# SuneelFreimuth/raytracer-server

Measured on NVIDIA B200. Metric: samples/sec (Mrays/sec alongside) on flying_unicorn, higher is better.
Workload: dtype f32

## Files before the change

### raytracer-server_b200/csrc/wavefront.cuh

```cuda
#pragma once

#include "adaptive_rule.cuh"
#include "intersect.cuh"
#include "octree.cuh"
#include "shade.cuh"

namespace rtb {

constexpr int WF_THREADS = 256;
constexpr int TILE = 32;
constexpr uint32_t SHADOW_PROBE = 0x80000000u;
constexpr uint32_t MAX_DEPTH_FIELD = 4095u;
constexpr uint32_t FETCH_CHUNK = 32;
constexpr int REFILL_BELOW = 28;
#ifndef RTB_PARK_BELOW
#define RTB_PARK_BELOW 20
#endif
#ifndef RTB_SHADE_CHUNK
#define RTB_SHADE_CHUNK 64
#endif
constexpr uint32_t SHADE_CHUNK = RTB_SHADE_CHUNK;
constexpr int SHADE_PARK_BELOW = RTB_PARK_BELOW;
constexpr uint32_t SHADE_SEG = 128;
constexpr uint32_t HIT_HOLE = 0xffffffffu;
// ... 391 lines not shown
        const unsigned idle_mask = __ballot_sync(0xffffffffu, idle);
        if (idle_mask && !exhausted) {
            if (!warp_reserve(&C->cursor_trav, count, wnext, wend)) exhausted = true;
            else {
                const uint32_t pos = wnext + __popc(idle_mask & ((1u << lane) - 1u));
                if (idle && pos < wend) {
                    const uint32_t my = perm ? perm[pos] : pos;
                    if (my < n_ext) {
                        const float2 h2 = Q.hit[my];
                        if (__float_as_uint(h2.y) != HIT_HOLE) {
                            slot = my;
                            kind = 0;
                            const float4 o4 = Q.o[my], d4 = Q.d[my];
                            trav_begin(a.S, T, f3(o4), f3(d4), __float_as_uint(o4.w), h2.x);
                        }
                    } else {
                        const float4 d4 = SQ.d[my - n_ext];
                        if (__float_as_uint(d4.w) != TLIM_HOLE) {
                            slot = my - n_ext;
                            const float4 o4 = SQ.o[slot];
                            kind = (__float_as_uint(SQ.c[slot].w) & SHADOW_PROBE) ? 2 : 1;
                            occluded = false;
                            trav_begin(a.S, T, f3(o4), f3(d4), __float_as_uint(o4.w), d4.w);
                        }
                    }
                }
                if (COUNT && lane == 0) { dbg[4] += 1; dbg[5] += min((uint32_t)__popc(idle_mask), wend - wnext); }
                wnext = min(wnext + (uint32_t)__popc(idle_mask), wend);
            }
        }
        const unsigned active = __ballot_sync(0xffffffffu, T.node != NODE_SENTINEL);
        if (active == 0) {
            if (exhausted) break;
            continue;
        }
        for (;;) {
            int trips = 0;
            if (!COUNT && steps == INNER_STEPS) {
#pragma unroll
                for (int k = 0; k < INNER_STEPS; ++k) {
                    if (T.node < 0) break;
                    trav_inner<COUNT>(a.S, T, sbase, sstride, lstack, work);
                }
            } else {
                for (int k = 0; k < steps && T.node >= 0; ++k) {
                    trav_inner<COUNT>(a.S, T, sbase, sstride, lstack, work);
                    ++trips;
                }
            }
            if (COUNT) {
                int mx = trips;
                for (int off = 16; off; off >>= 1) mx = max(mx, __shfl_xor_sync(0xffffffffu, mx, off));
                const unsigned lm = __ballot_sync(0xffffffffu, T.node < 0 && T.node != NODE_SENTINEL);
                if (lane == 0) { dbg[0] += 1; dbg[1] += 32ull * mx; dbg[2] += lm ? 1 : 0; dbg[3] += __popc(lm); }
            }
            if (T.node < 0 && T.node != NODE_SENTINEL) {
                trav_leaf<false, COUNT>(a.S, T, work);
                if (kind == 1 && T.best_id != PC_NONE) {
                    occluded = true;
                    T.node = NODE_SENTINEL;
                } else {
                    trav_pop(T, sbase, sstride, lstack);
                }
            }
            const unsigned act = __ballot_sync(0xffffffffu, T.node != NODE_SENTINEL);
            if (act == 0 || (!exhausted && __popc(act) < refill_below)) break;
        }
    }
    if (COUNT) {
        for (int off = 16; off; off >>= 1) {
            work[0] += __shfl_down_sync(0xffffffffu, work[0], off);
            work[1] += __shfl_down_sync(0xffffffffu, work[1], off);
        }
        if (lane == 0) {
            atomicAdd(&C->node_visits, (unsigned long long)work[0]);
            atomicAdd(&C->tri_tests, (unsigned long long)work[1]);
            for (int k = 0; k < 6; ++k) atomicAdd(&C->dbg[k], dbg[k]);
        }
    }
}

enum : int { OCT_IDLE = 0, OCT_NEXT_MESH, OCT_DESCEND, OCT_LEAF, OCT_DONE };
constexpr int OCT_STEPS = 12;

template <bool COUNT>
__global__ void __launch_bounds__(WF_THREADS, 4) k_traverse_octree(const __grid_constant__ RenderArgs a, int c) {
    extern __shared__ __align__(16) unsigned char smem_raw[];
    int2* const nstack = reinterpret_cast<int2*>(smem_raw) + threadIdx.x;
    const unsigned nstride = blockDim.x;
    DevCtrl* C = a.ctrl;
    const uint32_t n_ext = min(C->ext_head(c), a.Pcap);
    const uint32_t count = n_ext + min(C->sh_head(c), a.SPcap);
    const unsigned lane = threadIdx.x & 31;
    const int light_obj = a.S.hdr->light_obj;
    const uint32_t* const perm = a.bin_bits > 0 ? a.bin_perm : nullptr;
    const int refill_below = a.tune_refill > 0 ? a.tune_refill : REFILL_BELOW;
    const int steps = a.tune_steps > 0 ? a.tune_steps : OCT_STEPS;
    const float4* const N = a.S.oct_nodes;
    uint32_t work[2] = {0, 0};
    const uint32_t gwarp = (blockIdx.x * blockDim.x + threadIdx.x) >> 5;
    uint32_t wnext = min(gwarp * FETCH_CHUNK, count), wend = min(gwarp * FETCH_CHUNK + FETCH_CHUNK, count);
    bool exhausted = false;
    if (blockIdx.x * (WF_THREADS / 32) * FETCH_CHUNK >= count) return;
    float3 o = f3(0.f, 0.f, 0.f), d = o, inv = o;
    uint32_t origin = 0, best_id = PC_NONE, slot = 0, order = 0;
    float best_t = 0.f;
    uint2 obytes = make_uint2(0u, 0u);
    uint32_t rem = 0;
    int level = 0, mesh = -1, leaf_first = 0, leaf_cnt = 0;
    int cur_base = 0, cur_mask = 0;
    int phase = OCT_IDLE, kind = -1;

    for (;;) {
        if (phase == OCT_DONE) {
            if (kind == 0) {
                if (best_id != PC_NONE) a.qin.hit[slot] = make_float2(best_t, __uint_as_float(best_id));
            } else {
                const float4 c4 = a.sqin.c[slot];
                bool add;
                if (kind == 2) add = best_id != PC_NONE && __float_as_int(__ldg(a.S.tris + (size_t)(best_id - TRI_BASE) * TRI_STRIDE + 2).w) == light_obj;
                else add = best_id == PC_NONE;
                if (add) accum_add(a.accum, __float_as_uint(c4.w) & ~SHADOW_PROBE, f3(c4));
            }
            phase = OCT_IDLE;
            kind = -1;
        }
        const unsigned idle_mask = __ballot_sync(0xffffffffu, phase == OCT_IDLE);
        if (idle_mask && !exhausted) {
            if (!warp_reserve(&C->cursor_trav, count, wnext, wend)) exhausted = true;
            else {
                const uint32_t q = wnext + __popc(idle_mask & ((1u << lane) - 1u));
                if (phase == OCT_IDLE && q < wend) {
                    const uint32_t my = perm ? perm[q] : q;
                    float4 o4, d4;
                    bool take = false;
                    if (my < n_ext) {
                        const float2 h2 = a.qin.hit[my];
                        if (__float_as_uint(h2.y) != HIT_HOLE) {
                            take = true;
                            slot = my;
                            kind = 0;
                            o4 = a.qin.o[my];
                            d4 = a.qin.d[my];
                            best_t = h2.x;
                        }
                    } else {
                        d4 = a.sqin.d[my - n_ext];
                        if (__float_as_uint(d4.w) != TLIM_HOLE) {
                            take = true;
                            slot = my - n_ext;
                            o4 = a.sqin.o[slot];
                            kind = (__float_as_uint(a.sqin.c[slot].w) & SHADOW_PROBE) ? 2 : 1;
                            best_t = d4.w;
                        }
                    }
                    if (take) {
                        o = f3(o4);
                        d = f3(d4);
                        inv = f3(1.0f / d.x, 1.0f / d.y, 1.0f / d.z);
                        origin = __float_as_uint(o4.w);
                        best_id = PC_NONE;
                        mesh = -1;
                        phase = OCT_NEXT_MESH;
                    }
                }
                wnext = min(wnext + (uint32_t)__popc(idle_mask), wend);
            }
        }
        if (__ballot_sync(0xffffffffu, phase != OCT_IDLE) == 0) {
            if (exhausted) break;
            continue;
        }
        for (;;) {
            if (phase == OCT_NEXT_MESH) {
                int root = -1;
                if (!(kind == 1 && best_id != PC_NONE))
                    while (++mesh < a.S.n_oct_meshes && (root = __ldg(a.S.oct_roots + mesh)) < 0) {}
                if (root < 0) phase = OCT_DONE;
                else {
                    const float4 rmn = __ldg(N + (size_t)root * 2), rmx = __ldg(N + (size_t)root * 2 + 1);
                    if (__float_as_int(rmx.w) >= 0) {
                        leaf_first = __float_as_int(rmn.w);
                        leaf_cnt = __float_as_int(rmx.w);
                        level = -1;
                        phase = OCT_LEAF;
                    } else {
                        order = oct_search_order(rmn, rmx, o);
                        obytes = oct_order_bytes(order);
                        level = 0;
                        cur_base = __float_as_int(rmn.w);
                        cur_mask = -1 - __float_as_int(rmx.w);
                        rem = oct_present_in_order(cur_mask, obytes);
                        phase = OCT_DESCEND;
                    }
                }
            }
            for (int k = 0; k < steps; ++k) {
                if (!__any_sync(0xffffffffu, phase == OCT_DESCEND)) break;
                if (phase != OCT_DESCEND) continue;
                if (rem == 0u) {
                    if (level == 0) phase = OCT_NEXT_MESH;
                    else {
                        --level;
                        const int2 up = nstack[level * nstride];
                        cur_base = up.x;
                        cur_mask = up.y & 255;
                        rem = (unsigned)up.y >> 8;
                    }
                    continue;
                }
                const unsigned p = (unsigned)__ffs((int)rem) - 1u;
                rem &= rem - 1u;
                const int i = (int)(order >> (3 * p)) & 7;
                const int ch = cur_base + __popc((unsigned)cur_mask & ((1u << i) - 1u));
                const float4 cmn = __ldg(N + (size_t)ch * 2), cmx = __ldg(N + (size_t)ch * 2 + 1);
                if (COUNT) work[0]++;
                if (!oct_box_hit(cmn, cmx, o, d, inv)) continue;
                const int cnt = __float_as_int(cmx.w);
                if (cnt >= 0) {
                    leaf_first = __float_as_int(cmn.w);
                    leaf_cnt = cnt;
                    phase = OCT_LEAF;
                } else if (level + 1 < OCT_MAX_DEPTH) {
                    nstack[level * nstride] = make_int2(cur_base, cur_mask | (int)(rem << 8));
                    ++level;
                    cur_base = __float_as_int(cmn.w);
                    cur_mask = -1 - cnt;
                    rem = oct_present_in_order(cur_mask, obytes);
                }
            }
            if (__any_sync(0xffffffffu, phase == OCT_LEAF)) {
                const bool owner_lane = phase == OCT_LEAF;
                const int my_cnt = owner_lane ? leaf_cnt : 0;
                if (COUNT) work[1] += (uint32_t)my_cnt;
                int incl = my_cnt;
#pragma unroll
                for (int off = 1; off < 32; off <<= 1) {
                    const int v = __shfl_up_sync(0xffffffffu, incl, off);
                    if ((int)lane >= off) incl += v;
                }
                const int total = __shfl_sync(0xffffffffu, incl, 31);
                const int excl = incl - my_cnt;
                float bt = INFINITY;
                uint32_t bid = PC_NONE;
                for (int base = 0; base < total; base += 32) {
                    const int pair = base + (int)lane;
                    int own = 0;
#pragma unroll
                    for (int step = 16; step; step >>= 1) {
                        const int cand = own + step;
                        const int e = __shfl_sync(0xffffffffu, excl, cand & 31);
                        if (e <= pair) own = cand;
                    }
                    const int k_in = pair - __shfl_sync(0xffffffffu, excl, own);
                    const float3 ro = f3(__shfl_sync(0xffffffffu, o.x, own), __shfl_sync(0xffffffffu, o.y, own), __shfl_sync(0xffffffffu, o.z, own));
                    const float3 rd = f3(__shfl_sync(0xffffffffu, d.x, own), __shfl_sync(0xffffffffu, d.y, own), __shfl_sync(0xffffffffu, d.z, own));
                    const uint32_t rorigin = __shfl_sync(0xffffffffu, origin, own);
                    const int rfirst = __shfl_sync(0xffffffffu, leaf_first, own);
                    float t = INFINITY;
                    uint32_t id = PC_NONE;
                    if (pair < total) {
                        float tt;
                        uint32_t ii;
                        if (oct_tri_test(a.S, rfirst + k_in, ro, rd, rorigin, tt, ii)) { t = tt; id = ii; }
                    }
#pragma unroll
                    for (int off = 1; off < 32; off <<= 1) {
                        const float t2 = __shfl_down_sync(0xffffffffu, t, off);
                        const uint32_t i2 = __shfl_down_sync(0xffffffffu, id, off);
                        const int o2 = __shfl_down_sync(0xffffffffu, own, off);
                        if ((int)lane + off < 32 && o2 == own && t2 < t) { t = t2; id = i2; }
                    }
                    const int src = max(excl - base, 0);
                    const float ts = __shfl_sync(0xffffffffu, t, src & 31);
                    const uint32_t is = __shfl_sync(0xffffffffu, id, src & 31);
                    if (owner_lane && excl < base + 32 && excl + my_cnt > base && ts < bt) { bt = ts; bid = is; }
                }
                if (owner_lane) {
                    if (bid != PC_NONE) {
                        if (bt < best_t) {
                            best_t = bt;
                            best_id = bid;
                        }
                        phase = OCT_NEXT_MESH;
                    } else phase = level < 0 ? OCT_NEXT_MESH : OCT_DESCEND;
                }
            }
            const unsigned act = __ballot_sync(0xffffffffu, phase != OCT_DONE && phase != OCT_IDLE);
            if (act == 0 || (!exhausted && __popc(act) < refill_below)) break;
        }
    }
    if (COUNT) {
        for (int off = 16; off; off >>= 1) {
            work[0] += __shfl_down_sync(0xffffffffu, work[0], off);
            work[1] += __shfl_down_sync(0xffffffffu, work[1], off);
        }
        if (lane == 0) {
            atomicAdd(&C->node_visits, (unsigned long long)work[0]);
            atomicAdd(&C->tri_tests, (unsigned long long)work[1]);
        }
    }
}

constexpr uint32_t SEG_NEXT = 0x80000000u;
struct ShadeSegs {
    uint32_t base[3];
    uint32_t used[3];
};
template <int DIR>
__device__ __forceinline__ uint32_t seg_alloc(ShadeSegs& W, uint32_t& nb, unsigned cls, uint32_t* ctr, unsigned mask, unsigned lane) {
    uint32_t base = W.base[cls], used = W.used[cls];
    bool has_next = used & SEG_NEXT;
    used &= ~SEG_NEXT;
    const uint32_t n = __popc(mask);
    const uint32_t r = used + __popc(mask & ((1u << lane) - 1u));
    const uint32_t step = (uint32_t)(DIR * (int)SHADE_SEG);
    uint32_t slot;
    if (used + n > SHADE_SEG) {
        if (!has_next && lane == cls) nb = atomic_add_lane(ctr, step);
        uint32_t nbase = __shfl_sync(0xffffffffu, nb, cls);
        if (DIR < 0) nbase -= 1u;
        slot = r < SHADE_SEG ? base + (uint32_t)(DIR * (int)r) : nbase + (uint32_t)(DIR * (int)(r - SHADE_SEG));
        base = nbase;
        used = used + n - SHADE_SEG;
        has_next = false;
    } else {
        slot = base + (uint32_t)(DIR * (int)r);
        used += n;
    }
    if (!has_next && used + 64u > SHADE_SEG) {
        if (lane == cls) nb = atomic_add_lane(ctr, step);
        has_next = true;
    }
    __syncwarp();
    W.base[cls] = base;
    W.used[cls] = used | (has_next ? SEG_NEXT : 0u);
    return slot;
}
template <int DIR>
__device__ __forceinline__ uint32_t seg_slot(uint32_t base, uint32_t k) { return base + (uint32_t)(DIR * (int)k); }

constexpr int SHADE_THREADS_NOMESH = 160;
constexpr int SHADE_THREADS_NEE = 160;
constexpr int shade_cta(int mode, bool mesh = true) { return !mesh ? SHADE_THREADS_NOMESH : (mode == 1 ? SHADE_THREADS_NEE : SHADE_THREADS); }
template <int MODE, int NP = 0, int NS = 0, bool MESH = true, int THREADS = SHADE_THREADS, bool INLINE = false>
__global__ void __launch_bounds__(THREADS, THREADS == SHADE_THREADS ? RTB_SHADE_MINB : 640 / THREADS) k_shade(const __grid_constant__ RenderArgs a, int c) {
    constexpr bool FAST = MODE != 0;
    extern __shared__ __align__(16) unsigned char smem_raw[];
    DevCtrl* C = a.ctrl;
    const DevSceneHeader* hdr = a.S.hdr;
    const uint32_t head = C->ext_head(c), tail = C->ext_tail(c);
    const uint32_t count = head + (a.Pcap - tail);
    if (blockIdx.x * (THREADS / 32) * SHADE_CHUNK >= count) return;
    const SharedScene sh = stage_scene(a.S, smem_raw, INLINE);
    const unsigned lane = threadIdx.x & 31;
    const unsigned below = (1u << lane) - 1u;
    const PathQueue &Q = a.qin, &N = a.qout;
    const int light_obj = hdr->light_obj;
    const bool light_is_mesh = FAST ? false : hdr->light_geom == 2;
    const bool mis = MODE == 1 ? false : (MODE == 2 ? true : a.estimator == 1);
    const bool mis2 = FAST ? false : a.estimator == 2;
    const bool probe_mode = FAST ? false : a.probe_px != nullptr;
    const float3 Le = f3(sh.mats[light_obj].emitted);
    const int n_prims = a.S.n_prims, n_planes = a.S.n_planes;
    const ShadowQueue& SQ = a.sqout;
    uint32_t* const ctr_front = &C->ext_head(1 - c);
    uint32_t* const ctr_back = &C->ext_tail(1 - c);
    uint32_t* const ctr_sh = &C->sh_head(1 - c);
    uint32_t n_ext = 0, n_ext_bvh = 0, n_sh = 0, n_sh_bvh = 0, n_queued = 0;
    uint32_t n_sh_inline = 0;
    auto slot_of = [&](uint32_t i) { return i < head ? i : tail + (i - head); };

    const uint32_t gwarp = (blockIdx.x * THREADS + threadIdx.x) >> 5;
    uint32_t wnext = min(gwarp * SHADE_CHUNK, count), wend = min(gwarp * SHADE_CHUNK + SHADE_CHUNK, count);
    bool exhausted = count <= a.shade_warps * SHADE_CHUNK;
    const bool big_launch = count > a.shade_warps * SHADE_CHUNK * 8u;
    uint32_t nbase = 0;
    if (!exhausted && lane == 0) nbase = atomic_add_lane(&C->cursor_shade, SHADE_CHUNK);

    __shared__ __align__(16) float4 spare[5][THREADS];
    const uint32_t sp_o = (uint32_t)__cvta_generic_to_shared(&spare[0][threadIdx.x]);
    constexpr uint32_t SP_D = THREADS * 16u, SP_B = 2u * SP_D, SP_N = 3u * SP_D, SP_H = 4u * SP_D;
    bool cur_valid = false, cont = false, sp_valid = false, sp_nrm = false;
    float2 h2 = make_float2(0.f, __uint_as_float(PC_NONE));
    float4 o4 = make_float4(0, 0, 0, 0), d4 = o4, b4 = o4, tri_n = o4;
    float4 ev_keep = o4;
    uint32_t cur_slot = 0, sp_slot = 0;
    __shared__ ShadeSegs segs[THREADS / 32];
    ShadeSegs& W = segs[threadIdx.x >> 5];
    if (lane < 3) {
        W.base[lane] = 0;
        W.used[lane] = SHADE_SEG;
    }
    __syncwarp();
    uint32_t nb = 0;
    bool sh_tight = false;

    for (;;) {
        if (!cur_valid && sp_valid) {
            cp_async_wait_all();
            h2 = lds_f2(sp_o + SP_H);
            o4 = lds_f4(sp_o);
            d4 = lds_f4(sp_o + SP_D);
            b4 = lds_f4(sp_o + SP_B);
            cur_slot = sp_slot;
            const uint32_t idn = __float_as_uint(h2.y);
            if (idn != PC_NONE && idn != HIT_HOLE && idn >= TRI_BASE)
                tri_n = sp_nrm ? lds_f4(sp_o + SP_N) : __ldg(a.S.tri_nrm + (idn - TRI_BASE));
            cur_valid = idn != HIT_HOLE;
            cont = false;
            sp_valid = false;
        }
        {
            const unsigned need = __ballot_sync(0xffffffffu, !sp_valid);
            if (need && wnext < wend) {
                const uint32_t my = wnext + __popc(need & below);
                if (!sp_valid && my < wend) {
                    sp_slot = slot_of(my);
                    cp_async8(sp_o + SP_H, Q.hit + sp_slot);
                    cp_async16(sp_o, Q.o + sp_slot);
                    cp_async16(sp_o + SP_D, Q.d + sp_slot);
                    cp_async16(sp_o + SP_B, Q.beta + sp_slot);
                    cp_async_commit();
                    sp_valid = true;
                    sp_nrm = false;
                }
                wnext = min(wnext + (uint32_t)__popc(need), wend);
            }
            if (wnext >= wend && !exhausted) {
                const uint32_t b = __shfl_sync(0xffffffffu, nbase, 0);
                if (b >= count) exhausted = true;
                else {
                    wnext = b;
                    wend = min(b + SHADE_CHUNK, count);
                    if (lane == 0) nbase = atomic_add_lane(&C->cursor_shade, SHADE_CHUNK);
                }
            }
        }
        const unsigned have_work = __ballot_sync(0xffffffffu, cur_valid || sp_valid);
        const bool drained = wnext >= wend && exhausted;
        if (have_work == 0 && drained) break;
        const bool park = drained && big_launch && __popc(have_work) < SHADE_PARK_BELOW;

        bool ext_push = false, want_sh = false, pr_push = false, pr_try = false;
        float3 pos, nbeta;
        uint32_t pcode, eflags;
        float3 next_dir = f3(0.f, 0.f, 0.f), sh_dir = f3(0.f, 0.f, 0.f), sh_contrib;
        float sh_tlim = 0.f;
        float4 ev = make_float4(0.f, 0.f, 0.f, 0.f);
        float4 pd, pc;
        const uint32_t acc = __float_as_uint(d4.w);
        const uint32_t sdw = __float_as_uint(b4.w);

        if (cur_valid) {
            const uint32_t id = __float_as_uint(h2.y);
            if (id != PC_NONE) {
                const float t = h2.x;
                const float3 o = f3(o4), d = f3(d4);
                const uint32_t origin = __float_as_uint(o4.w);
                float3 beta = f3(b4);
                const uint32_t sample = sdw >> 12, depth = sdw & 0xfffu;
                const HitGeom hg = hit_geometry(sh, o, d, t, id, tri_n);
                pos = hg.pos;
                pcode = hg.pcode;
                const DevMaterial& mat = sh.mats[hg.obj];
                const float3 ovec = (origin & PC_STALE_O) ? (cont ? f3(INLINE ? ev_keep : tri_n) : f3(Q.ov[cur_slot])) : -d;
                const float3 emitted = f3(mat.emitted);
                const bool emits = emitted.x != 0.f || emitted.y != 0.f || emitted.z != 0.f;
                if (depth == 1u) {
                    if (emits) accum_add(a.accum, acc, beta * emitted);
                } else if (mis2 && (origin & PC_MIS_PENDING)) {
                    if (emits && hg.obj == light_obj) {
                        const float pdf_b = cont ? (INLINE ? ev_keep.w : tri_n.w) : Q.ov[cur_slot].w;
                        const float pdf_l = a.light_pdf * (t * t) / fmaxf(dot(hg.n, -d), 1e-20f);
                        accum_add(a.accum, acc, beta * emitted * (pdf_b / (pdf_b + pdf_l)));
                    }
                } else if (origin & PC_SPEC_PENDING) {
                    if (emits) accum_add(a.accum, acc, beta * emitted);
                    const DevMaterial& pm = sh.mats[object_of(a.S, sh, origin & PC_ID_MASK)];
                    const float inv_pp = (depth - 1u) <= 5u ? 1.0f : (1.0f / 0.9f);
                    beta = beta * f3(pm.k) * inv_pp;
                }
                const float p = depth <= 5u ? 1.0f : 0.9f;
                const float inv_p = depth <= 5u ? 1.0f : (1.0f / 0.9f);
                const uint32_t pidx = probe_mode && a.pixel_list ? acc >> 2 : acc;
                const uint32_t rng_pixel = probe_mode ? (uint32_t)(a.probe_py[pidx] * a.width + a.probe_px[pidx]) : acc >> 2;
                const bool dead_surface = mat.brdf == 0 && mat.k.x == 0.f && mat.k.y == 0.f && mat.k.z == 0.f;
                const bool dead_path = beta.x == 0.f && beta.y == 0.f && beta.z == 0.f;
                if (!dead_surface && !dead_path && depth < MAX_DEPTH_FIELD) {
                    const VertexRng vr = rng_vertex(rng_pixel, sample, depth, a.keys);
                    float lobe_u = 0.f, select_u = 0.f;
                    if (!FAST && (mat.brdf == 2 || light_is_mesh)) {
                        const float4 r1 = rng_block(rng_pixel, sample, depth, 1u, a.keys);
                        lobe_u = r1.x;
                        select_u = r1.y;
                    }
                    const float4 r0 = make_float4(vr.light_u1, vr.light_u2, vr.rr, select_u);
                    const float4 rb = make_float4(vr.brdf_u1, vr.brdf_u2, lobe_u, 0.f);
                    if (mat.brdf == 1) {
                        if (r0.z < p) {
                            next_dir = flip_across(ovec, hg.n);
                            ext_push = true;
                            eflags = hg.pcode | PC_SPEC_PENDING | PC_STALE_O;
                            nbeta = beta;
                            ev = make_float4(ovec.x, ovec.y, ovec.z, 0.f);
                        }
                    } else {
                        float3 y, ny;
                        float pdf_a;
                        if (FAST) light_sample_sphere(a.light_sphere, a.light_pdf, r0, y, ny, pdf_a);
                        else light_sample<FAST>(a.S, sh.prims, hdr, r0, y, ny, pdf_a);
                        float3 dv = y - hg.pos;
                        float r2 = dot(dv, dv);
                        float inv_dist = rsqrtf(r2);
                        float dist = r2 * inv_dist;
                        float3 inc = dv * inv_dist;
                        float3 f = brdf_eval<FAST>(mat, hg.n, ovec, inc);
                        float3 contrib;
                        if (!mis) {
                            float g = __fdividef(dot(hg.n, inc) * dot(ny, -inc), r2 * pdf_a);
                            contrib = beta * Le * f * g;
                            if (mis2 && mat.brdf == 0) {
                                const float pdf_l = pdf_a * r2 / fmaxf(fabsf(dot(ny, -inc)), 1e-20f);
                                const float pdf_b = fmaxf(dot(hg.n, inc), 0.f) * INV_PI_F;
                                contrib = contrib * (pdf_l / (pdf_l + pdf_b));
                            }
                        } else {
                            float pdf_light = pdf_a * (r2 / dot(ny, -inc));
                            float3 itmp;
                            float pdf_fresh;
                            brdf_sample<FAST>(mat, hg.n, inc, rng_block(rng_pixel, sample, depth, 2u, a.keys), itmp, pdf_fresh);
                            contrib = beta * Le * f * (dot(hg.n, inc) / (pdf_light + pdf_fresh));
                        }
                        if (contrib.x != 0.f || contrib.y != 0.f || contrib.z != 0.f) {
                            want_sh = true;
                            sh_dir = inc;
                            sh_tlim = dist - SHADOW_MARGIN;
                            sh_contrib = contrib;
                        }
                        if (mis) {
                            float3 i2;
                            float pdf2;
                            brdf_sample<FAST>(mat, hg.n, ovec, rng_block(rng_pixel, sample, depth, 4u, a.keys), i2, pdf2);
                            if (i2.x != 0.f || i2.y != 0.f || i2.z != 0.f) {
                                float3 y2, ny2;
                                float pdf_a2;
                                if (FAST) light_sample_sphere(a.light_sphere, a.light_pdf, rng_block(rng_pixel, sample, depth, 3u, a.keys), y2, ny2, pdf_a2);
                                else light_sample<FAST>(a.S, sh.prims, hdr, rng_block(rng_pixel, sample, depth, 3u, a.keys), y2, ny2, pdf_a2);
                                float3 dv2 = y2 - hg.pos;
                                float pdf_light2 = pdf_a2 * (dot(dv2, dv2) / dot(ny2, -i2));
                                float3 c2 = beta * Le * brdf_eval<FAST>(mat, hg.n, ovec, i2) * (dot(hg.n, i2) / (pdf2 + pdf_light2));
                                if (c2.x != 0.f || c2.y != 0.f || c2.z != 0.f) {
                                    pr_try = true;
                                    float ta;
                                    uint32_t ida;
                                    if (NP > 0 && NP < 8) analytic_closest_small<NP, NS>(a.ss, origin_group_of(sh, hg.pcode), hg.pos, i2, hg.pcode, ta, ida);
                                    else analytic_closest(sh, n_planes, n_prims, hg.pos, i2, hg.pcode, ta, ida);
                                    const bool needs_bvh = MESH ? ray_hits_bvh_box(a.S, hg.pos, i2, ta) : false;
                                    if (!light_is_mesh) {
                                        if (ida != PC_NONE && sh.prims[ida].obj == light_obj) {
                                            if (needs_bvh && INLINE) {
                                                ++n_sh_inline;
                                                uint32_t idt = PC_NONE;
                                                float tt = ta;
                                                if (!bvh_traverse<true, false>(a.S, sh, hg.pos, i2, hg.pcode, tt, idt, ta + SHADOW_MARGIN, nullptr)) accum_add(a.accum, acc, c2);
                                            } else if (needs_bvh) {
                                                pr_push = true;
                                                pd = make_float4(i2.x, i2.y, i2.z, ta);
                                                pc = make_float4(c2.x, c2.y, c2.z, __uint_as_float(acc));
                                            } else {
                                                accum_add(a.accum, acc, c2);
                                            }
                                        }
                                    } else if (needs_bvh && INLINE) {
                                        ++n_sh_inline;
                                        uint32_t idt = PC_NONE;
                                        float tt = ta;
                                        bvh_traverse<false, false>(a.S, sh, hg.pos, i2, hg.pcode, tt, idt, 0.f, nullptr);
                                        if (idt != PC_NONE && __float_as_int(__ldg(a.S.tris + (size_t)(idt - TRI_BASE) * TRI_STRIDE + 2).w) == light_obj) accum_add(a.accum, acc, c2);
                                    } else if (needs_bvh) {
                                        pr_push = true;
                                        pd = make_float4(i2.x, i2.y, i2.z, ta);
                                        pc = make_float4(c2.x, c2.y, c2.z, __uint_as_float(acc | SHADOW_PROBE));
                                    }
                                }
                            }
                        }
                        if (r0.z < p) {
                            float pdf1;
                            brdf_sample<FAST>(mat, hg.n, ovec, rb, next_dir, pdf1);
                            if (next_dir.x != 0.f || next_dir.y != 0.f || next_dir.z != 0.f) {
                                if (FAST || mat.brdf == 0) nbeta = beta * f3(mat.k) * inv_p;
                                else nbeta = beta * brdf_eval(mat, hg.n, ovec, next_dir) * (dot(hg.n, next_dir) / (pdf1 * p));
                                ext_push = true;
                                eflags = hg.pcode;
                                if (mis2 && mat.brdf == 0) {
                                    eflags = hg.pcode | PC_MIS_PENDING;
                                    ev = make_float4(0.f, 0.f, 0.f, pdf1);
                                }
                            }
                        }
                    }
                }
            }
        }
        uint32_t trip_sh = __popc(__ballot_sync(0xffffffffu, want_sh));
        unsigned mp = 0;
        if (mis) {
            trip_sh += __popc(__ballot_sync(0xffffffffu, pr_try));
            mp = __ballot_sync(0xffffffffu, pr_push);
            if (mp) {
                const uint32_t slot = seg_alloc<1>(W, nb, 2u, ctr_sh, mp, lane);
                if (pr_push) {
                    if (slot < a.SPcap) { SQ.o[slot] = make_float4(pos.x, pos.y, pos.z, __uint_as_float(pcode)); SQ.d[slot] = pd; SQ.c[slot] = pc; }
                    else atomicAdd(&C->overflow, 1u);
                }
                n_sh_bvh += __popc(mp);
            }
        }
        n_sh += trip_sh;

        float ta;
        uint32_t ida;
        bool ext_box = false;
        if (ext_push || want_sh) {
            bool occ, sh_box;
            if (NP == 8) analytic_pair_small8(a.ss, n_planes, n_prims, origin_group_of(sh, pcode), pos, pcode, next_dir, ta, ida, sh_dir, sh_tlim, occ);
            else if (NP > 0) analytic_pair_small<NP, NS>(a.ss, origin_group_of(sh, pcode), pos, pcode, next_dir, ta, ida, sh_dir, sh_tlim, occ);
            else analytic_pair(sh, n_planes, n_prims, pos, pcode, next_dir, ta, ida, sh_dir, sh_tlim, occ);
            if (MESH) ray_pair_hits_bvh_box(a.S, pos, next_dir, ta, sh_dir, sh_tlim, ext_box, sh_box);
            else ext_box = sh_box = false;
            if (want_sh) {
                want_sh = false;
                if (occ) {
                } else if (sh_box && INLINE) {
                    ++n_sh_inline;
                    uint32_t idt = PC_NONE;
                    float tt = sh_tlim;
                    if (!bvh_traverse<true, false>(a.S, sh, pos, sh_dir, pcode, tt, idt, sh_tlim + SHADOW_MARGIN, nullptr)) accum_add(a.accum, acc, sh_contrib);
                } else if (sh_box) {
                    want_sh = true;
                } else {
                    accum_add(a.accum, acc, sh_contrib);
                }
            }
        }
        const bool sh_push = want_sh;

        const unsigned ms = __ballot_sync(0xffffffffu, sh_push);
        if (ms) {
            const uint32_t slot = seg_alloc<1>(W, nb, 2u, ctr_sh, ms, lane);
            if (sh_push) {
                if (slot < a.SPcap) {
                    SQ.o[slot] = make_float4(pos.x, pos.y, pos.z, __uint_as_float(pcode));
                    SQ.d[slot] = make_float4(sh_dir.x, sh_dir.y, sh_dir.z, sh_tlim);
                    SQ.c[slot] = make_float4(sh_contrib.x, sh_contrib.y, sh_contrib.z, __uint_as_float(acc));
                } else {
                    atomicAdd(&C->overflow, 1u);
                }
            }
            n_sh_bvh += __popc(ms);
        }

        n_ext += __popc(__ballot_sync(0xffffffffu, ext_push));
        n_ext_bvh += __popc(__ballot_sync(0xffffffffu, ext_push && ext_box));
        if (INLINE && ext_push && ext_box) bvh_traverse<false, false>(a.S, sh, pos, next_dir, pcode, ta, ida, 0.f, nullptr);
        const bool ext_front = !INLINE && ext_box;
        bool keep = ext_push && !ext_front && !park && (!(sh_push || pr_push) || !sh_tight);
        if (ext_push && !ext_front && ida == PC_NONE) {
            keep = false;
            ext_push = false;
        }
        if (keep) ext_push = false;
        const unsigned mf = __ballot_sync(0xffffffffu, ext_push && ext_front);
        const unsigned mb = __ballot_sync(0xffffffffu, ext_push && !ext_front);
        if (mf | mb) {
            uint32_t slot = 0;
            if (mf) { const uint32_t v = seg_alloc<1>(W, nb, 0u, ctr_front, mf, lane); if (ext_front) slot = v; }
            if (mb) { const uint32_t v = seg_alloc<-1>(W, nb, 1u, ctr_back, mb, lane); if (!ext_front) slot = v; }
            if (ext_push && slot >= a.Pcap) { atomicAdd(&C->overflow, 1u); ext_push = false; }
            if (ext_push) {
                N.o[slot] = make_float4(pos.x, pos.y, pos.z, __uint_as_float(eflags));
                N.d[slot] = make_float4(next_dir.x, next_dir.y, next_dir.z, __uint_as_float(acc));
                N.beta[slot] = make_float4(nbeta.x, nbeta.y, nbeta.z, __uint_as_float(sdw + 1u));
                N.hit[slot] = make_float2(ta, __uint_as_float(ida));
                if (eflags & (PC_STALE_O | PC_MIS_PENDING)) N.ov[slot] = ev;
            }
            n_queued += __popc(__ballot_sync(0xffffffffu, ext_push));
        }
        if (ms | mp) sh_tight = W.base[2] + SHADE_SEG > a.SP;
        cur_valid = keep;
        if (keep) {
            o4 = make_float4(pos.x, pos.y, pos.z, __uint_as_float(eflags));
            d4 = make_float4(next_dir.x, next_dir.y, next_dir.z, __uint_as_float(acc));
            b4 = make_float4(nbeta.x, nbeta.y, nbeta.z, __uint_as_float(sdw + 1u));
            h2 = make_float2(ta, __uint_as_float(ida));
            if (INLINE) {
                ev_keep = ev;
                if (ida != PC_NONE && ida >= TRI_BASE) tri_n = __ldg(a.S.tri_nrm + (ida - TRI_BASE));
            } else {
                tri_n = ev;
            }
            cont = true;
        }
        if (sp_valid && !sp_nrm) {
            cp_async_wait_all();
            const uint32_t idn = __float_as_uint(lds_f2(sp_o + SP_H).y);
            if (idn == HIT_HOLE) sp_valid = false;
            else if (idn != PC_NONE && idn >= TRI_BASE) {
                cp_async16(sp_o + SP_N, a.S.tri_nrm + (idn - TRI_BASE));
                cp_async_commit();
            }
            sp_nrm = true;
        }
    }
    {
        const float2 hole = make_float2(0.f, __uint_as_float(HIT_HOLE));
        const float4 hole4 = make_float4(0.f, 0.f, 0.f, __uint_as_float(TLIM_HOLE));
        auto mark_path = [&](uint32_t slot) { if (slot < a.Pcap) N.hit[slot] = hole; else atomicAdd(&C->overflow, 1u); };
        auto mark_sh = [&](uint32_t slot) { if (slot < a.SPcap) SQ.d[slot] = hole4; else atomicAdd(&C->overflow, 1u); };
        const uint32_t fu = W.used[0] & ~SEG_NEXT, bu = W.used[1] & ~SEG_NEXT, su = W.used[2] & ~SEG_NEXT;
        for (uint32_t k = fu + lane; k < SHADE_SEG; k += 32) mark_path(seg_slot<1>(W.base[0], k));
        for (uint32_t k = bu + lane; k < SHADE_SEG; k += 32) mark_path(seg_slot<-1>(W.base[1], k));
        for (uint32_t k = su + lane; k < SHADE_SEG; k += 32) mark_sh(seg_slot<1>(W.base[2], k));
        const uint32_t nf = __shfl_sync(0xffffffffu, nb, 0), nbk = __shfl_sync(0xffffffffu, nb, 1) - 1u, ns = __shfl_sync(0xffffffffu, nb, 2);
        if (W.used[0] & SEG_NEXT) for (uint32_t k = lane; k < SHADE_SEG; k += 32) mark_path(seg_slot<1>(nf, k));
        if (W.used[1] & SEG_NEXT) for (uint32_t k = lane; k < SHADE_SEG; k += 32) mark_path(seg_slot<-1>(nbk, k));
        if (W.used[2] & SEG_NEXT) for (uint32_t k = lane; k < SHADE_SEG; k += 32) mark_sh(seg_slot<1>(ns, k));
    }
    if (INLINE)
        for (int off = 16; off; off >>= 1) n_sh_inline += __shfl_down_sync(0xffffffffu, n_sh_inline, off);
    if (lane == 0) {
        if (n_queued) { atomicAdd(&C->live[1 - c], n_queued); atomicAdd(&C->paths_queued, (unsigned long long)n_queued); }
        if (n_sh_bvh) atomicAdd(&C->sh_live[1 - c], n_sh_bvh);
        if (n_ext) atomicAdd(&C->rays_extension, (unsigned long long)n_ext);
        if (n_ext_bvh) atomicAdd(&C->rays_bvh, (unsigned long long)n_ext_bvh);
        if (n_sh) atomicAdd(&C->rays_shadow, (unsigned long long)n_sh);
        if (n_sh_bvh + n_sh_inline) atomicAdd(&C->shadow_bvh, (unsigned long long)(n_sh_bvh + n_sh_inline));
    }
}

__device__ __forceinline__ float clamp01_keep_nan(float x) { return x < 0.f ? 0.f : (x > 1.f ? 1.f : x); }
__device__ __forceinline__ unsigned char to_u8(float v) {
    if (!(v == v)) return 0;
    if (v <= 0.f) return 0;
    if (v >= 255.f) return 255;
    return (unsigned char)v;
}

__global__ void k_resolve(RenderArgs a, unsigned char* __restrict__ out_rgb8, float4* __restrict__ out_sub, int scanline) {
    int lp = blockIdx.x * blockDim.x + threadIdx.x;
    if (lp >= a.n_local_tiles * 1024) return;
    int x, y;
    bool in = local_to_xy(lp + a.tile_base * 1024, a.rank, a.world, a.tiles_x, a.width, a.height, x, y);
    float3 px = f3(0.f, 0.f, 0.f);
    if (in) {
        uint32_t p = (uint32_t)(y * a.width + x);
        const uint32_t ks_done = a.tile_ks ? a.tile_ks[(lp >> 10) + a.tile_base] : a.ks_done;
        for (int s = 0; s < 4; ++s) {
            uint32_t cnt = ks_done > (uint32_t)s ? (ks_done - (uint32_t)s + 3u) / 4u : 0u;
            float inv = cnt ? 1.0f / (float)cnt : 0.0f;
            float4 v = a.accum[p * 4u + s];
            if (out_sub) out_sub[(size_t)lp * 4 + s] = make_float4(v.x * inv, v.y * inv, v.z * inv, 0.f);
            px.x += clamp01_keep_nan(v.x * inv) * 0.25f;
            px.y += clamp01_keep_nan(v.y * inv) * 0.25f;
            px.z += clamp01_keep_nan(v.z * inv) * 0.25f;
        }
    } else if (out_sub) {
        for (int s = 0; s < 4; ++s) out_sub[(size_t)lp * 4 + s] = make_float4(0.f, 0.f, 0.f, 0.f);
    }
    unsigned char r = to_u8(powf(clamp01_keep_nan(px.x), 1.0f / 2.2f) * 255.0f + 0.5f);
    unsigned char g = to_u8(powf(clamp01_keep_nan(px.y), 1.0f / 2.2f) * 255.0f + 0.5f);
    unsigned char b = to_u8(powf(clamp01_keep_nan(px.z), 1.0f / 2.2f) * 255.0f + 0.5f);
    if (scanline) {
        if (!in) return;
        size_t o = ((size_t)y * a.width + x) * 3;
        out_rgb8[o] = r; out_rgb8[o + 1] = g; out_rgb8[o + 2] = b;
    } else {
        size_t o = (size_t)lp * 3;
        out_rgb8[o] = in ? r : 0; out_rgb8[o + 1] = in ? g : 0; out_rgb8[o + 2] = in ? b : 0;
    }
}

__global__ void k_resolve_list(const float4* __restrict__ accum, int n, int num_samples, float* __restrict__ out3) {
    int i = blockIdx.x * blockDim.x + threadIdx.x;
    if (i >= n) return;
    const float inv = num_samples > 0 ? 1.0f / (float)num_samples : 0.0f;
    float3 px = f3(0.f, 0.f, 0.f);
    for (int s = 0; s < 4; ++s) {
        const float4 v = accum[(size_t)i * 4 + s];
        px.x += clamp01_keep_nan(v.x * inv) * 0.25f;
        px.y += clamp01_keep_nan(v.y * inv) * 0.25f;
        px.z += clamp01_keep_nan(v.z * inv) * 0.25f;
    }
    out3[3 * i] = powf(clamp01_keep_nan(px.x), 1.0f / 2.2f) * 255.0f + 0.5f;
    out3[3 * i + 1] = powf(clamp01_keep_nan(px.y), 1.0f / 2.2f) * 255.0f + 0.5f;
    out3[3 * i + 2] = powf(clamp01_keep_nan(px.z), 1.0f / 2.2f) * 255.0f + 0.5f;
}

struct AdaptArgs {
    float4* accum;
    float2* mom;
    int32_t* list;
    uint32_t* tile_ks;
    float* tile_err;
    int width, height, tiles_x;
    int pass_spp, spp, min_spp;
    float target;
};

constexpr int ADAPT_THREADS = 256;
constexpr int COMPACT_THREADS = 1024;

__global__ void k_adapt_init(AdaptArgs a, int n_tiles) {
    const int t = blockIdx.x * blockDim.x + threadIdx.x;
    if (t >= n_tiles) return;
    a.list[t] = t;
    a.tile_ks[t] = 0u;
    a.tile_err[t] = 0.0f;
}

__global__ void __launch_bounds__(ADAPT_THREADS) k_adapt(AdaptArgs a) {
    __shared__ float warp_max[ADAPT_THREADS / 32];
    const int t = a.list[blockIdx.x];
    const uint32_t ks = a.tile_ks[t] + (uint32_t)a.pass_spp;
    const int B = (int)(ks / (uint32_t)a.pass_spp);
    const float inv_n = 4.0f / (float)a.pass_spp;
    float err = 0.0f;
    for (int slot = threadIdx.x; slot < 1024; slot += ADAPT_THREADS) {
        int x, y;
        if (!local_to_xy(t * 1024 + slot, 0, 1, a.tiles_x, a.width, a.height, x, y)) continue;
        const uint32_t p = (uint32_t)(y * a.width + x);
        float4 sub[4];
        for (int s = 0; s < 4; ++s) sub[s] = a.accum[p * 4u + s];
        float2 mom = a.mom[p];
        err = fmaxf(err, adapt_pixel(sub, inv_n, mom, B));
        for (int s = 0; s < 4; ++s) a.accum[p * 4u + s].w = sub[s].w;
        a.mom[p] = mom;
    }
    for (int off = 16; off; off >>= 1) err = fmaxf(err, __shfl_xor_sync(0xffffffffu, err, off));
    if ((threadIdx.x & 31) == 0) warp_max[threadIdx.x >> 5] = err;
    __syncthreads();
    if (threadIdx.x == 0) {
        for (int w = 1; w < ADAPT_THREADS / 32; ++w) err = fmaxf(err, warp_max[w]);
        a.tile_ks[t] = ks;
        a.tile_err[t] = err;
        const bool go_on = ks < (uint32_t)a.spp && (ks < (uint32_t)a.min_spp || a.target <= 0.0f || err > a.target);
        if (!go_on) a.list[blockIdx.x] = -1;
    }
}

__global__ void __launch_bounds__(COMPACT_THREADS) k_compact_tiles(int32_t* list, int n, volatile int* host_count) {
    __shared__ int warp_sum[COMPACT_THREADS / 32];
    __shared__ int base;
    const unsigned lane = threadIdx.x & 31, w = threadIdx.x >> 5;
    if (threadIdx.x == 0) base = 0;
    __syncthreads();
    for (int c0 = 0; c0 < n; c0 += COMPACT_THREADS) {
        const int i = c0 + (int)threadIdx.x;
        const int32_t v = i < n ? list[i] : -1;
        const unsigned keep = __ballot_sync(0xffffffffu, v >= 0);
        if (lane == 0) warp_sum[w] = __popc(keep);
        __syncthreads();
        int before = base, total = 0;
        for (int k = 0; k < COMPACT_THREADS / 32; ++k) {
            before += k < (int)w ? warp_sum[k] : 0;
            total += warp_sum[k];
        }
        if (v >= 0) list[before + __popc(keep & ((1u << lane) - 1u))] = v;
        __syncthreads();
        if (threadIdx.x == 0) base += total;
        __syncthreads();
    }
    if (threadIdx.x == 0) {
        *host_count = base;
        __threadfence_system();
    }
}

__global__ void k_untile(const unsigned char* __restrict__ shards, long long shard_stride, int world, int tiles_x, int tiles_y,
                         int width, int height, unsigned char* __restrict__ frame) {
    long long g = (long long)blockIdx.x * blockDim.x + threadIdx.x;
    long long total = (long long)tiles_x * tiles_y * 1024;
    if (g >= total) return;
    int t = (int)(g >> 10), slot = (int)(g & 1023);
    int rank = t % world, lt = t / world;
    int x, y;
    if (!local_to_xy(lt * 1024 + slot, rank, world, tiles_x, width, height, x, y)) return;
    const unsigned char* s = shards + (size_t)rank * shard_stride + ((size_t)lt * 1024 + slot) * 3;
    size_t o = ((size_t)y * width + x) * 3;
    frame[o] = s[0]; frame[o + 1] = s[1]; frame[o + 2] = s[2];
}

template <bool COUNT>
__global__ void __launch_bounds__(WF_THREADS) k_trace_rays(DevScene S, long long n, const float* __restrict__ org, const float* __restrict__ dir,
                                                           const Camera cam, int width, int height, int sx, int sy, float dx, float dy,
                                                           int32_t* __restrict__ obj, int32_t* __restrict__ tri, float* __restrict__ tout,
                                                           unsigned long long* __restrict__ work_out, int accel = 0) {
    extern __shared__ __align__(16) unsigned char smem_raw[];
    const SharedScene sh = stage_scene(S, smem_raw);
    uint32_t work[2] = {0, 0};
    for (long long i = (long long)blockIdx.x * blockDim.x + threadIdx.x; i < n; i += (long long)gridDim.x * blockDim.x) {
        float3 o, d;
        if (org) {
            o = f3(org[3 * i], org[3 * i + 1], org[3 * i + 2]);
            d = f3(dir[3 * i], dir[3 * i + 1], dir[3 * i + 2]);
        } else {
            int y = (int)(i / width), x = (int)(i - (long long)y * width);
            o = cam.pos;
            d = camera_dir(cam, x, height - y - 1, sx, sy, dx, dy, (float)width, (float)height);
        }
        float t;
        uint32_t id;
        analytic_closest(sh, S.n_planes, S.n_prims, o, d, PC_NONE, t, id);
        if (accel == 1) {
            oct_trace_meshes(S, o, d, PC_NONE, t, id, COUNT ? work : nullptr);
        } else if (ray_hits_bvh_box(S, o, d, t)) {
            bvh_traverse<false, COUNT>(S, sh, o, d, PC_NONE, t, id, 0.0f, work);
        }
        if (id == PC_NONE) {
            obj[i] = -1; tri[i] = -1; tout[i] = INFINITY;
        } else if (id < TRI_BASE) {
            obj[i] = sh.prims[id].obj; tri[i] = -1; tout[i] = t;
        } else {
            const float4* tp = S.tris + (size_t)(id - TRI_BASE) * TRI_STRIDE;
            int ob = __float_as_int(__ldg(tp + 2).w);
            obj[i] = ob;
            tri[i] = __float_as_int(__ldg(tp + 1).w) - sh.mats[ob].first_tri;
            tout[i] = t;
        }
    }
    if (COUNT && work_out) {
        atomicAdd(&work_out[0], (unsigned long long)work[0]);
        atomicAdd(&work_out[1], (unsigned long long)work[1]);
    }
}

__global__ void k_fma_peak(float* out, int iters) {
    float a0 = threadIdx.x * 1e-3f, a1 = a0 + 1.f, a2 = a0 + 2.f, a3 = a0 + 3.f, a4 = a0 + 4.f, a5 = a0 + 5.f, a6 = a0 + 6.f, a7 = a0 + 7.f;
    const float m = 0.999f, c = 1e-3f;
    for (int i = 0; i < iters; ++i) {
#pragma unroll
        for (int u = 0; u < 8; ++u) {
            a0 = fmaf(a0, m, c); a1 = fmaf(a1, m, c); a2 = fmaf(a2, m, c); a3 = fmaf(a3, m, c);
            a4 = fmaf(a4, m, c); a5 = fmaf(a5, m, c); a6 = fmaf(a6, m, c); a7 = fmaf(a7, m, c);
        }
    }
    out[blockIdx.x * blockDim.x + threadIdx.x] = a0 + a1 + a2 + a3 + a4 + a5 + a6 + a7;
}

}
```

Baseline: 1.029 billion.

## Move shade queue segment allocator into per-lane registers with fused reservation

Replaces the shared-memory per-warp segment allocator (three separate seg_alloc calls, each with its own ballots, shuffles and syncwarp) with a register-resident per-lane state where lanes 0-2 own the front, back and shadow classes and a single seg_reserve call serves all three. Per-trip counters are also folded into one lane-distributed tally reduced by shuffles at the end. Overflow handling now decrements live and paths_queued. The aim is fewer ballots, shared-memory round trips and atomics in the shade loop, at the cost of more intricate slot arithmetic with one's-complement back-queue indexing.

New measurement: 1.041 billion, median of 6. +1.2%, better.

```diff
diff --git a/raytracer-server_b200/csrc/wavefront.cuh b/raytracer-server_b200/csrc/wavefront.cuh
--- a/raytracer-server_b200/csrc/wavefront.cuh
+++ b/raytracer-server_b200/csrc/wavefront.cuh
@@ -717,43 +717,53 @@
     }
 }
 
+constexpr uint32_t SEG_ROOM = 0x1ffu;
+constexpr int SEG_CLASS_SHIFT = 29;
 constexpr uint32_t SEG_NEXT = 0x80000000u;
-struct ShadeSegs {
-    uint32_t base[3];
-    uint32_t used[3];
+struct SegLane {
+    uint32_t next;
+    uint32_t room;
+    uint32_t nb;
 };
-template <int DIR>
-__device__ __forceinline__ uint32_t seg_alloc(ShadeSegs& W, uint32_t& nb, unsigned cls, uint32_t* ctr, unsigned mask, unsigned lane) {
-    uint32_t base = W.base[cls], used = W.used[cls];
-    bool has_next = used & SEG_NEXT;
-    used &= ~SEG_NEXT;
-    const uint32_t n = __popc(mask);
-    const uint32_t r = used + __popc(mask & ((1u << lane) - 1u));
-    const uint32_t step = (uint32_t)(DIR * (int)SHADE_SEG);
-    uint32_t slot;
-    if (used + n > SHADE_SEG) {
-        if (!has_next && lane == cls) nb = atomic_add_lane(ctr, step);
-        uint32_t nbase = __shfl_sync(0xffffffffu, nb, cls);
-        if (DIR < 0) nbase -= 1u;
-        slot = r < SHADE_SEG ? base + (uint32_t)(DIR * (int)r) : nbase + (uint32_t)(DIR * (int)(r - SHADE_SEG));
-        base = nbase;
-        used = used + n - SHADE_SEG;
-        has_next = false;
-    } else {
-        slot = base + (uint32_t)(DIR * (int)r);
-        used += n;
-    }
-    if (!has_next && used + 64u > SHADE_SEG) {
-        if (lane == cls) nb = atomic_add_lane(ctr, step);
+static_assert(offsetof(DevCtrl, ext_tail_) - offsetof(DevCtrl, ext_head_) == 256 && offsetof(DevCtrl, sh_head_) - offsetof(DevCtrl, ext_tail_) == 256,
+              "seg_reserve addresses class k's counter as ext_head(i) + 64 k");
+static_assert(SHADE_SEG >= 96 && SHADE_SEG <= SEG_ROOM, "one atomic per class and trip");
+struct SegSlots {
+    uint32_t path, sh;
+};
+__device__ __forceinline__ SegSlots seg_reserve(SegLane& S, uint32_t* ctr_front, uint32_t n, unsigned mf, unsigned mb, unsigned ms,
+                                                bool front, unsigned lane) {
+    const uint32_t room = S.room & SEG_ROOM, cls = (S.room >> SEG_CLASS_SHIFT) & 3u;
+    bool has_next = S.room & SEG_NEXT;
+    if (lane < 3 && n != 0 && !has_next && n + 64u > room) {
+        S.nb = atomic_add_lane(ctr_front + 64 * cls, cls == 1 ? 0u - SHADE_SEG : SHADE_SEG);
         has_next = true;
     }
-    __syncwarp();
-    W.base[cls] = base;
-    W.used[cls] = used | (has_next ? SEG_NEXT : 0u);
-    return slot;
-}
-template <int DIR>
-__device__ __forceinline__ uint32_t seg_slot(uint32_t base, uint32_t k) { return base + (uint32_t)(DIR * (int)k); }
+    const uint32_t x = S.next;
+    uint32_t y = x, next = x + n, left = room - n;
+    const bool over = lane < 3 && n > room;
+    if (__any_sync(0xffffffffu, over)) {
+        if (over) {
+            y = (cls == 1 ? 0u - S.nb : S.nb) - room;
+            next = y + n;
+            left = SHADE_SEG + room - n;
+            has_next = false;
+        }
+    }
+    S.next = next;
+    S.room = left | (cls << SEG_CLASS_SHIFT) | (has_next ? SEG_NEXT : 0u);
+    const unsigned below = (1u << lane) - 1u;
+    const uint32_t ks = __popc(ms & below), ts = __shfl_sync(0xffffffffu, room, 2);
+    const uint32_t xs = __shfl_sync(0xffffffffu, x, 2), ys = __shfl_sync(0xffffffffu, y, 2);
+    const unsigned pl = front ? 0u : 1u;
+    const uint32_t kp = __popc((front ? mf : mb) & below), tp = __shfl_sync(0xffffffffu, room, pl);
+    const uint32_t xp = __shfl_sync(0xffffffffu, x, pl), yp = __shfl_sync(0xffffffffu, y, pl);
+    const uint32_t p = (kp < tp ? xp : yp) + kp;
+    SegSlots r;
+    r.sh = (ks < ts ? xs : ys) + ks;
+    r.path = front ? p : ~p;
+    return r;
+}
 
 constexpr int SHADE_THREADS_NOMESH = 160;
 constexpr int SHADE_THREADS_NEE = 160;
@@ -780,9 +790,7 @@
     const int n_prims = a.S.n_prims, n_planes = a.S.n_planes;
     const ShadowQueue& SQ = a.sqout;
     uint32_t* const ctr_front = &C->ext_head(1 - c);
-    uint32_t* const ctr_back = &C->ext_tail(1 - c);
-    uint32_t* const ctr_sh = &C->sh_head(1 - c);
-    uint32_t n_ext = 0, n_ext_bvh = 0, n_sh = 0, n_sh_bvh = 0, n_queued = 0;
+    uint32_t tally = 0;
     uint32_t n_sh_inline = 0;
     auto slot_of = [&](uint32_t i) { return i < head ? i : tail + (i - head); };
 
@@ -801,14 +809,7 @@
     float4 o4 = make_float4(0, 0, 0, 0), d4 = o4, b4 = o4, tri_n = o4;
     float4 ev_keep = o4;
     uint32_t cur_slot = 0, sp_slot = 0;
-    __shared__ ShadeSegs segs[THREADS / 32];
-    ShadeSegs& W = segs[threadIdx.x >> 5];
-    if (lane < 3) {
-        W.base[lane] = 0;
-        W.used[lane] = SHADE_SEG;
-    }
-    __syncwarp();
-    uint32_t nb = 0;
+    SegLane segs = {0u, (lane & 3u) << SEG_CLASS_SHIFT, 0u};
     bool sh_tight = false;
 
     for (;;) {
@@ -1019,25 +1020,24 @@
                 }
             }
         }
-        uint32_t trip_sh = __popc(__ballot_sync(0xffffffffu, want_sh));
         unsigned mp = 0;
         if (mis) {
-            trip_sh += __popc(__ballot_sync(0xffffffffu, pr_try));
+            const unsigned mt = __ballot_sync(0xffffffffu, pr_try);
             mp = __ballot_sync(0xffffffffu, pr_push);
+            const uint32_t n = __popc(lane == 2 ? mp : (lane == 4 ? mt : 0u));
+            tally += n;
             if (mp) {
-                const uint32_t slot = seg_alloc<1>(W, nb, 2u, ctr_sh, mp, lane);
+                const uint32_t slot = seg_reserve(segs, ctr_front, n, 0u, 0u, mp, false, lane).sh;
                 if (pr_push) {
                     if (slot < a.SPcap) { SQ.o[slot] = make_float4(pos.x, pos.y, pos.z, __uint_as_float(pcode)); SQ.d[slot] = pd; SQ.c[slot] = pc; }
                     else atomicAdd(&C->overflow, 1u);
                 }
-                n_sh_bvh += __popc(mp);
-            }
-        }
-        n_sh += trip_sh;
+            }
+        }
 
         float ta;
         uint32_t ida;
-        bool ext_box = false;
+        bool ext_box = false, sh_push = false;
         if (ext_push || want_sh) {
             bool occ, sh_box;
             if (NP == 8) analytic_pair_small8(a.ss, n_planes, n_prims, origin_group_of(sh, pcode), pos, pcode, next_dir, ta, ida, sh_dir, sh_tlim, occ);
@@ -1046,7 +1046,6 @@
             if (MESH) ray_pair_hits_bvh_box(a.S, pos, next_dir, ta, sh_dir, sh_tlim, ext_box, sh_box);
             else ext_box = sh_box = false;
             if (want_sh) {
-                want_sh = false;
                 if (occ) {
                 } else if (sh_box && INLINE) {
                     ++n_sh_inline;
@@ -1054,56 +1053,60 @@
                     float tt = sh_tlim;
                     if (!bvh_traverse<true, false>(a.S, sh, pos, sh_dir, pcode, tt, idt, sh_tlim + SHADOW_MARGIN, nullptr)) accum_add(a.accum, acc, sh_contrib);
                 } else if (sh_box) {
-                    want_sh = true;
+                    sh_push = true;
                 } else {
                     accum_add(a.accum, acc, sh_contrib);
                 }
             }
         }
-        const bool sh_push = want_sh;
-
-        const unsigned ms = __ballot_sync(0xffffffffu, sh_push);
-        if (ms) {
-            const uint32_t slot = seg_alloc<1>(W, nb, 2u, ctr_sh, ms, lane);
-            if (sh_push) {
-                if (slot < a.SPcap) {
-                    SQ.o[slot] = make_float4(pos.x, pos.y, pos.z, __uint_as_float(pcode));
-                    SQ.d[slot] = make_float4(sh_dir.x, sh_dir.y, sh_dir.z, sh_tlim);
-                    SQ.c[slot] = make_float4(sh_contrib.x, sh_contrib.y, sh_contrib.z, __uint_as_float(acc));
-                } else {
-                    atomicAdd(&C->overflow, 1u);
-                }
-            }
-            n_sh_bvh += __popc(ms);
-        }
-
-        n_ext += __popc(__ballot_sync(0xffffffffu, ext_push));
-        n_ext_bvh += __popc(__ballot_sync(0xffffffffu, ext_push && ext_box));
-        if (INLINE && ext_push && ext_box) bvh_traverse<false, false>(a.S, sh, pos, next_dir, pcode, ta, ida, 0.f, nullptr);
+
+        if (INLINE) {
+            const unsigned mt = __ballot_sync(0xffffffffu, ext_push && ext_box);
+            if (lane == 0) tally += __popc(mt);
+            if (ext_push && ext_box) bvh_traverse<false, false>(a.S, sh, pos, next_dir, pcode, ta, ida, 0.f, nullptr);
+        }
         const bool ext_front = !INLINE && ext_box;
+        const unsigned me = __ballot_sync(0xffffffffu, ext_push);
         bool keep = ext_push && !ext_front && !park && (!(sh_push || pr_push) || !sh_tight);
         if (ext_push && !ext_front && ida == PC_NONE) {
             keep = false;
             ext_push = false;
         }
         if (keep) ext_push = false;
-        const unsigned mf = __ballot_sync(0xffffffffu, ext_push && ext_front);
+        constexpr bool QUEUED = MESH && !INLINE;
+        const unsigned ms = QUEUED ? __ballot_sync(0xffffffffu, sh_push) : 0u;
+        const unsigned mf = QUEUED ? __ballot_sync(0xffffffffu, ext_push && ext_front) : 0u;
         const unsigned mb = __ballot_sync(0xffffffffu, ext_push && !ext_front);
-        if (mf | mb) {
-            uint32_t slot = 0;
-            if (mf) { const uint32_t v = seg_alloc<1>(W, nb, 0u, ctr_front, mf, lane); if (ext_front) slot = v; }
-            if (mb) { const uint32_t v = seg_alloc<-1>(W, nb, 1u, ctr_back, mb, lane); if (!ext_front) slot = v; }
-            if (ext_push && slot >= a.Pcap) { atomicAdd(&C->overflow, 1u); ext_push = false; }
+        const unsigned mw = __ballot_sync(0xffffffffu, want_sh);
+        const unsigned m03 = lane & 2 ? (lane & 1 ? me : ms) : (lane & 1 ? mb : mf);
+        const uint32_t n = __popc(lane & 4 ? mw : m03);
+        tally += n;
+        if (mf | mb | ms) {
+            const SegSlots slot = seg_reserve(segs, ctr_front, n, mf, mb, ms, ext_front, lane);
+            if (QUEUED && sh_push) {
+                if (slot.sh < a.SPcap) {
+                    SQ.o[slot.sh] = make_float4(pos.x, pos.y, pos.z, __uint_as_float(pcode));
+                    SQ.d[slot.sh] = make_float4(sh_dir.x, sh_dir.y, sh_dir.z, sh_tlim);
+                    SQ.c[slot.sh] = make_float4(sh_contrib.x, sh_contrib.y, sh_contrib.z, __uint_as_float(acc));
+                } else {
+                    atomicAdd(&C->overflow, 1u);
+                }
+            }
+            if (ext_push && slot.path >= a.Pcap) {
+                atomicAdd(&C->overflow, 1u);
+                atomicSub(&C->live[1 - c], 1u);
+                atomicAdd(&C->paths_queued, ~0ull);
+                ext_push = false;
+            }
             if (ext_push) {
-                N.o[slot] = make_float4(pos.x, pos.y, pos.z, __uint_as_float(eflags));
-                N.d[slot] = make_float4(next_dir.x, next_dir.y, next_dir.z, __uint_as_float(acc));
-                N.beta[slot] = make_float4(nbeta.x, nbeta.y, nbeta.z, __uint_as_float(sdw + 1u));
-                N.hit[slot] = make_float2(ta, __uint_as_float(ida));
-                if (eflags & (PC_STALE_O | PC_MIS_PENDING)) N.ov[slot] = ev;
-            }
-            n_queued += __popc(__ballot_sync(0xffffffffu, ext_push));
-        }
-        if (ms | mp) sh_tight = W.base[2] + SHADE_SEG > a.SP;
+                N.o[slot.path] = make_float4(pos.x, pos.y, pos.z, __uint_as_float(eflags));
+                N.d[slot.path] = make_float4(next_dir.x, next_dir.y, next_dir.z, __uint_as_float(acc));
+                N.beta[slot.path] = make_float4(nbeta.x, nbeta.y, nbeta.z, __uint_as_float(sdw + 1u));
+                N.hit[slot.path] = make_float2(ta, __uint_as_float(ida));
+                if (eflags & (PC_STALE_O | PC_MIS_PENDING)) N.ov[slot.path] = ev;
+            }
+        }
+        if (ms | mp) sh_tight = __shfl_sync(0xffffffffu, segs.next + (segs.room & SEG_ROOM), 2) > a.SP;
         cur_valid = keep;
         if (keep) {
             o4 = make_float4(pos.x, pos.y, pos.z, __uint_as_float(eflags));
@@ -1132,19 +1135,28 @@
     {
         const float2 hole = make_float2(0.f, __uint_as_float(HIT_HOLE));
         const float4 hole4 = make_float4(0.f, 0.f, 0.f, __uint_as_float(TLIM_HOLE));
-        auto mark_path = [&](uint32_t slot) { if (slot < a.Pcap) N.hit[slot] = hole; else atomicAdd(&C->overflow, 1u); };
-        auto mark_sh = [&](uint32_t slot) { if (slot < a.SPcap) SQ.d[slot] = hole4; else atomicAdd(&C->overflow, 1u); };
-        const uint32_t fu = W.used[0] & ~SEG_NEXT, bu = W.used[1] & ~SEG_NEXT, su = W.used[2] & ~SEG_NEXT;
-        for (uint32_t k = fu + lane; k < SHADE_SEG; k += 32) mark_path(seg_slot<1>(W.base[0], k));
-        for (uint32_t k = bu + lane; k < SHADE_SEG; k += 32) mark_path(seg_slot<-1>(W.base[1], k));
-        for (uint32_t k = su + lane; k < SHADE_SEG; k += 32) mark_sh(seg_slot<1>(W.base[2], k));
-        const uint32_t nf = __shfl_sync(0xffffffffu, nb, 0), nbk = __shfl_sync(0xffffffffu, nb, 1) - 1u, ns = __shfl_sync(0xffffffffu, nb, 2);
-        if (W.used[0] & SEG_NEXT) for (uint32_t k = lane; k < SHADE_SEG; k += 32) mark_path(seg_slot<1>(nf, k));
-        if (W.used[1] & SEG_NEXT) for (uint32_t k = lane; k < SHADE_SEG; k += 32) mark_path(seg_slot<-1>(nbk, k));
-        if (W.used[2] & SEG_NEXT) for (uint32_t k = lane; k < SHADE_SEG; k += 32) mark_sh(seg_slot<1>(ns, k));
-    }
-    if (INLINE)
-        for (int off = 16; off; off >>= 1) n_sh_inline += __shfl_down_sync(0xffffffffu, n_sh_inline, off);
+        for (unsigned k = 0; k < 3; ++k) {
+            const uint32_t next = __shfl_sync(0xffffffffu, segs.next, k), room = __shfl_sync(0xffffffffu, segs.room, k);
+            const uint32_t nb = __shfl_sync(0xffffffffu, segs.nb, k), ahead = k == 1 ? 0u - nb : nb;
+            auto mark = [&](uint32_t idx) {
+                const uint32_t slot = k == 1 ? ~idx : idx;
+                if (slot < (k == 2 ? a.SPcap : a.Pcap)) {
+                    if (k == 2) SQ.d[slot] = hole4;
+                    else N.hit[slot] = hole;
+                } else {
+                    atomicAdd(&C->overflow, 1u);
+                }
+            };
+            for (uint32_t i = lane; i < (room & SEG_ROOM); i += 32) mark(next + i);
+            if (room & SEG_NEXT)
+                for (uint32_t i = lane; i < SHADE_SEG; i += 32) mark(ahead + i);
+        }
+    }
+    if (INLINE) n_sh_inline = __reduce_add_sync(0xffffffffu, n_sh_inline);
+    const uint32_t n_ext_bvh = __shfl_sync(0xffffffffu, tally, 0);
+    const uint32_t n_queued = (INLINE ? 0u : n_ext_bvh) + __shfl_sync(0xffffffffu, tally, 1);
+    const uint32_t n_sh_bvh = __shfl_sync(0xffffffffu, tally, 2);
+    const uint32_t n_ext = __shfl_sync(0xffffffffu, tally, 3), n_sh = __shfl_sync(0xffffffffu, tally, 4);
     if (lane == 0) {
         if (n_queued) { atomicAdd(&C->live[1 - c], n_queued); atomicAdd(&C->paths_queued, (unsigned long long)n_queued); }
         if (n_sh_bvh) atomicAdd(&C->sh_live[1 - c], n_sh_bvh);
```
